# HumanCompatibleAI/overcooked_ai

Hardware: NVIDIA H100
Metric: env-steps/sec (joint transitions) (higher is better)
Workload: dtype int32

## Files before the change

### overcooked_ai_b200/csrc/ovc_b200.cu

```cuda
#include <cuda.h>
#include <cuda_runtime.h>
#include <stdint.h>
#include <stdio.h>
#include <stdlib.h>
#include <string.h>

#include "../../include/ovc_b200.h"
#include "ovc_step.cuh"

namespace ovc {

static thread_local char g_err[512] = "";

static int fail(int code, const char *msg) {
    snprintf(g_err, sizeof g_err, "%s", msg);
    return code;
}
static int fail(int code, const char *msg, long long value) {
    snprintf(g_err, sizeof g_err, "%s (got %lld)", msg, value);
    return code;
}
static int cuda_fail(cudaError_t e, const char *what) {
    snprintf(g_err, sizeof g_err, "%s: %s", what, cudaGetErrorString(e));
    return OVC_E_CUDA;
}

__device__ __forceinline__ uint32_t smem_u32(const void *p) { return (uint32_t)__cvta_generic_to_shared(p); }

__device__ __forceinline__ void mbar_init(uint64_t *bar, int count) {
    asm volatile("mbarrier.init.shared::cta.b64 [%0], %1;" ::"r"(smem_u32(bar)), "r"(count) : "memory");
    asm volatile("fence.mbarrier_init.release.cluster;" ::: "memory");
    asm volatile("fence.proxy.async.shared::cta;" ::: "memory");
}
__device__ __forceinline__ void mbar_expect_tx(uint64_t *bar, uint32_t bytes) {
    asm volatile("mbarrier.arrive.expect_tx.shared::cta.b64 _, [%0], %1;" ::"r"(smem_u32(bar)), "r"(bytes) : "memory");
}
__device__ __forceinline__ void mbar_wait(uint64_t *bar, uint32_t parity) {
    uint32_t ok;
    do {
// ... 988 lines not shown
```

### overcooked_ai_b200/csrc/ovc_encfc.cuh

```cuda
#pragma once
#include <cuda_bf16.h>
#include <type_traits>

namespace ovc {

constexpr int EL_DYN = 19;
constexpr int EL_THREADS = 1024;
constexpr int EL_MAX_LAYOUTS = 8;
constexpr int EL_MAX_MEMBERS = 64;

struct EncLinArgs {
    const ovc_layout_t *layouts;
    const int32_t *state;
    const int32_t *view_swap;
    const __nv_bfloat16 *wt;
    const float *bias;
    __nv_bfloat16 *out;
    long long n_envs;
    int n_layouts, S, W, H, horizon, n_out, n_workers;
    float neg_slope;
    int seat;
    const int32_t *rows;
    const int32_t *range;
};
// ... 65 lines not shown
    constexpr int CS = 32 * CPL;
    extern __shared__ __align__(16) char el_smem[];
    const int WH = a.W * a.H;
    const int n_rows = WH * EL_DYN;
    __nv_bfloat16 *tab = reinterpret_cast<__nv_bfloat16 *>(el_smem);
    float *bias_eff = reinterpret_cast<float *>(el_smem + (size_t)n_rows * CS * 2);
    float *urg = bias_eff + a.n_layouts * CS;
    int *cook = reinterpret_cast<int *>(urg + CS);
    int *nslots = cook + a.n_layouts * 16;
    unsigned short *srow = reinterpret_cast<unsigned short *>(nslots + a.n_layouts * 2);

    const int n_slices = a.n_out / CS;
    const __nv_bfloat16 *wt = a.wt;
    const float *bias = a.bias;
    long long r_beg = 0, r_end = a.n_envs;
    int slice = blockIdx.x % n_slices, worker = blockIdx.x / n_slices;
    if constexpr (GROUPED) {
        int bx = blockIdx.x;
        const int per = n_slices * a.n_workers, k = bx / per;
        bx -= k * per;
        wt += (size_t)k * a.W * a.H * N_PLANES * a.n_out, bias += (size_t)k * a.n_out;
        r_beg = min(max((long long)__ldg(offsets + k), 0ll), a.n_envs);
        r_end = max(min((long long)__ldg(offsets + k + 1), a.n_envs), r_beg);
        slice = bx % n_slices, worker = bx / n_slices;
    }
    const int col0 = slice * CS;
    if constexpr (ROWS) {
        r_beg = max(__ldg(a.range), 0);
        r_end = min((long long)__ldg(a.range + 1), a.n_envs);
        if (r_beg + (long long)worker * (EL_THREADS / 32) >= r_end) return;
    }
    if constexpr (MASKED) {
        if ((long long)worker * (EL_THREADS / 32) >= r_end) return;
    }
    if constexpr (GROUPED) {
        if (r_beg + (long long)worker * (EL_THREADS / 32) >= r_end) return;
    }

    unsigned char *tplane = reinterpret_cast<unsigned char *>(srow + a.n_layouts * 128);
    for (int i = threadIdx.x; i < a.n_layouts * WH; i += EL_THREADS) {
        const int l = i / WH, cell = i - l * WH, x = cell / a.H, y = cell - x * a.H;
        tplane[l * 256 + cell] = (unsigned char)((0x000F0A0E0D0C0B00ull >> ((a.layouts[l].cell[(y << 4) | x] & 7) * 8)) & 0xFF);
    }
    __syncthreads();
    {
        constexpr int CH = CS * 2 / 16;
        for (int i = threadIdx.x; i < n_rows * CH; i += EL_THREADS) {
            const int r = i / CH, c = i - r * CH;
            const int cell = r / EL_DYN, d = r - cell * EL_DYN;
            const int plane = d < 10 ? d : d + 6;
            const uint4 *src = reinterpret_cast<const uint4 *>(wt + (size_t)(cell * N_PLANES + plane) * a.n_out + col0) + c;
            reinterpret_cast<uint4 *>(tab)[i] = __ldg(src);
// ... 15 lines not shown
            if (l == a.n_layouts) urg[c] = s;
            else bias_eff[i] = s;
        }
        for (int i = threadIdx.x; i < a.n_layouts * 128; i += EL_THREADS) {
            const ovc_layout_t *L = a.layouts + (i >> 7);
            const int pb = L->slot_pos[i & 127];
            srow[i] = (unsigned short)((((pb & 15) * a.H + (pb >> 4)) * EL_DYN) & 0xFFFF);
        }
        for (int i = threadIdx.x; i < a.n_layouts * 16; i += EL_THREADS) cook[i] = a.layouts[i >> 4].cook_time[i & 15];
        for (int i = threadIdx.x; i < a.n_layouts; i += EL_THREADS) {
            nslots[2 * i] = a.layouts[i].n_slots;
            nslots[2 * i + 1] = a.layouts[i].n_pots;
        }
    }
    __syncthreads();

    const int lane = threadIdx.x & 31, warp = threadIdx.x >> 5;
    constexpr int NW = EL_THREADS / 32;
    const __nv_bfloat16 *tab_lane = tab + lane * CPL;
    const long long stride = (long long)a.n_workers * NW;
    const int max_slot_chunks = (a.S - 4 + 31) / 32;

    for (long long r = r_beg + (long long)worker * NW + warp; r < r_end; r += stride) {
        long long env, row0 = 0;
        int vmask = 3;
        if constexpr (MASKED) {
            const int entry = __ldg(list + r);
            env = entry >> 2, vmask = entry & 3;
            if (!vmask) continue;
            row0 = __ldg(first + r);
// ... 151 lines not shown
    a.out = (__nv_bfloat16 *)out, a.n_envs = n_envs, a.n_layouts = n_layouts, a.S = S, a.W = W, a.H = H, a.horizon = horizon;
    a.n_out = n_out, a.neg_slope = neg_slope, a.seat = seat, a.rows = rows, a.range = range;
    const int n_slices = n_out / (32 * cpl);
    const long long want = (n_envs + EL_THREADS / 32 - 1) / (EL_THREADS / 32);
    int workers = n_sm / n_slices;
    if (grouped) workers /= n_members;
    if (workers < 1) workers = 1;
    if (workers > want) workers = (int)want;
    a.n_workers = workers;
    const size_t smem = encode_linear_smem(cpl, n_rows, n_layouts);
    cudaError_t e;
#define OVC_LAUNCH_EL(C, ...)                                                                                                 \
    do {                                                                                                                      \
        e = cudaFuncSetAttribute(encode_linear_kernel<C, __VA_ARGS__>, cudaFuncAttributeMaxDynamicSharedMemorySize, (int)smem); \
        if (e != cudaSuccess) return cuda_fail(e, "encode_linear kernel attribute");                                          \
        encode_linear_kernel<C, __VA_ARGS__><<<(unsigned)(workers * n_slices), EL_THREADS, smem, st>>>(a);                    \
    } while (0)
#define OVC_LAUNCH_ELM(C)                                                                                                     \
    do {                                                                                                                      \
        e = cudaFuncSetAttribute(encode_linear_masked_kernel<C>, cudaFuncAttributeMaxDynamicSharedMemorySize, (int)smem);     \
        if (e != cudaSuccess) return cuda_fail(e, "encode_linear kernel attribute");                                          \
        encode_linear_masked_kernel<C><<<(unsigned)(workers * n_slices), EL_THREADS, smem, st>>>(a, list, first);             \
    } while (0)
#define OVC_LAUNCH_ELG(C)                                                                                                     \
    do {                                                                                                                      \
        e = cudaFuncSetAttribute(encode_linear_grouped_kernel<C>, cudaFuncAttributeMaxDynamicSharedMemorySize, (int)smem);    \
        if (e != cudaSuccess) return cuda_fail(e, "encode_linear kernel attribute");                                          \
        encode_linear_grouped_kernel<C><<<grid, EL_THREADS, smem, st>>>(a, offsets);                                          \
    } while (0)
#define OVC_LAUNCH_ELGM(C)                                                                                                    \
    do {                                                                                                                      \
        e = cudaFuncSetAttribute(encode_linear_grouped_masked_kernel<C>, cudaFuncAttributeMaxDynamicSharedMemorySize, (int)smem); \
        if (e != cudaSuccess) return cuda_fail(e, "encode_linear kernel attribute");                                          \
        encode_linear_grouped_masked_kernel<C><<<grid, EL_THREADS, smem, st>>>(a, list, first, offsets);                      \
    } while (0)
    if (grouped && masked) {
        const unsigned grid = (unsigned)(workers * n_slices * n_members);
        if (cpl == 8) OVC_LAUNCH_ELGM(8);
        else if (cpl == 4) OVC_LAUNCH_ELGM(4);
        else OVC_LAUNCH_ELGM(2);
    } else if (grouped) {
        const unsigned grid = (unsigned)(workers * n_slices * n_members);
        if (cpl == 8) OVC_LAUNCH_ELG(8);
        else if (cpl == 4) OVC_LAUNCH_ELG(4);
        else OVC_LAUNCH_ELG(2);
    } else if (masked) {
        if (cpl == 8) OVC_LAUNCH_ELM(8);
        else if (cpl == 4) OVC_LAUNCH_ELM(4);
        else OVC_LAUNCH_ELM(2);
// ... 2 lines not shown
        else if (cpl == 4) OVC_LAUNCH_EL(4, true, true);
        else OVC_LAUNCH_EL(2, true, true);
    } else if (seat >= 0) {
        if (cpl == 8) OVC_LAUNCH_EL(8, true);
        else if (cpl == 4) OVC_LAUNCH_EL(4, true);
        else OVC_LAUNCH_EL(2, true);
    } else {
        if (cpl == 8) OVC_LAUNCH_EL(8, false);
        else if (cpl == 4) OVC_LAUNCH_EL(4, false);
        else OVC_LAUNCH_EL(2, false);
    }
#undef OVC_LAUNCH_EL
#undef OVC_LAUNCH_ELM
#undef OVC_LAUNCH_ELG
#undef OVC_LAUNCH_ELGM
    e = cudaGetLastError();
    if (e != cudaSuccess) return cuda_fail(e, "encode_linear kernel launch");
    return OVC_OK;
}

constexpr int WG_SMEM_LIMIT = 227 * 1024;

struct EncWgradArgs {
    const ovc_layout_t *layouts;
    const int32_t *state;
    const int32_t *swap;
    const float *dz;
    float *dwt;
    long long n_rec;
    int n_layouts, S, W, H, horizon, n_out, n_workers;
    int seat;
// ... 226 lines not shown
            counter[0] = step + 1;
            __threadfence();
        }
    }
}

enum class RowMap { Identity, View, Rows, Joint };

template <bool LOGP, RowMap MAP>
__global__ void __launch_bounds__(256) sample_actions_kernel(const float *__restrict__ scores, int ld, int n_actions, long long n_rows,
                                                             unsigned long long seed, unsigned long long *counter,
                                                             int32_t *__restrict__ actions, float *__restrict__ logp,
                                                             const int32_t *__restrict__ swap, int seat, const int32_t *__restrict__ rows,
                                                             const int32_t *__restrict__ range) {
    static_assert(MAP != RowMap::Joint, "the draw has no joint-rows form");
    const unsigned long long step = *reinterpret_cast<volatile unsigned long long *>(counter);
    const long long row = (long long)blockIdx.x * blockDim.x + threadIdx.x;
    const bool in = MAP == RowMap::Rows ? row >= max(__ldg(range), 0) && row < min((long long)__ldg(range + 1), n_rows) : row < n_rows;
    if (in) {
        const float *s = scores + row * ld;
        long long g = row;
        if constexpr (MAP != RowMap::Identity) {
            const long long e = MAP == RowMap::Rows ? (long long)__ldg(rows + row) : row;
            g = 2 * e + (seat ^ (swap && swap[e] != 0));
        }
        const uint32_t c3 = (uint32_t)(step >> 32) << 1;
        const Philox4 A = philox4x32_10(seed, (uint32_t)g, (uint32_t)((unsigned long long)g >> 32), (uint32_t)step, c3);
        Philox4 B = A;
        if (n_actions > 4) B = philox4x32_10(seed, (uint32_t)g, (uint32_t)((unsigned long long)g >> 32), (uint32_t)step, c3 | 1u);
        int best = 0;
// ... 88 lines not shown
    } else if (rewards) {
        reinterpret_cast<float2 *>(rewards)[e] = make_float2(__fadd_rn((float)sp, __fmul_rn(f, (float)sh.x)), __fadd_rn((float)sp, __fmul_rn(f, (float)sh.y)));
    }
    if (dones) dones[e] = done[e] != 0;
    if constexpr (STATS)
        episode_stats_update(stats, e, n_envs, sh, __fadd_rn((float)sp, __fmul_rn(f, (float)sh.x)), __fadd_rn((float)sp, __fmul_rn(f, (float)sh.y)),
                             done[e] != 0);
}

template <bool STATS>
__global__ void __launch_bounds__(256) accumulate_returns_kernel(const int32_t *__restrict__ sparse, const int32_t *__restrict__ shaped,
                                                                 float factor, long long n_envs, long long *__restrict__ ret_sparse,
                                                                 float *__restrict__ ret_mixed, const float *__restrict__ factor_dev,
                                                                 const int32_t *__restrict__ done, float *__restrict__ rewards,
                                                                 uint8_t *__restrict__ dones, const ovc_episode_stats_t stats) {
    const long long e = (long long)blockIdx.x * blockDim.x + threadIdx.x;
    if (e >= n_envs) return;
    record_body<STATS, false>(e, sparse, shaped, factor_dev ? *factor_dev : factor, n_envs, ret_sparse, ret_mixed, done, nullptr, 0, rewards,
                              dones, stats);
}

static int sample_actions_impl(const float *scores, int ld, int n_actions, long long n_rows, unsigned long long seed,
                               unsigned long long *counter, int32_t *actions, float *logp, cudaStream_t st, RowMap map = RowMap::Identity,
                               const int32_t *swap = nullptr, int seat = 0, const int32_t *rows = nullptr, const int32_t *range = nullptr) {
    const bool listed = map == RowMap::Rows;
    if (!scores || !counter || !actions || (listed && (!rows || !range))) return fail(OVC_E_BADARG, "null pointer argument");
    if (listed && seat != 0 && seat != 1) return fail(OVC_E_BADARG, "seat must be 0 or 1", seat);
    if (n_actions < 1 || n_actions > 8 || ld < n_actions) return fail(OVC_E_BADARG, "n_actions must be 1..8 and <= ld", n_actions);
    if (n_rows < 0) return fail(OVC_E_BADARG, "negative row count");
    if (listed) {
        if ((((uintptr_t)scores | (uintptr_t)actions | (uintptr_t)logp | (uintptr_t)swap | (uintptr_t)rows | (uintptr_t)range) & 3) != 0)
            return fail(OVC_E_BADARG, "scores, actions, logp, swap, rows and range must be 4-byte aligned");
        if (((uintptr_t)counter & 7) != 0) return fail(OVC_E_BADARG, "counter must be 8-byte aligned");
    } else if (map == RowMap::View && (((uintptr_t)scores | (uintptr_t)actions | (uintptr_t)logp | (uintptr_t)swap) & 3) != 0) {
        return fail(OVC_E_BADARG, "scores, actions, logp and swap must be 4-byte aligned");
    }
    if (n_rows == 0) return OVC_OK;
    const unsigned grid = (unsigned)((n_rows + 255) / 256);
    auto kern = listed                ? (logp ? sample_actions_kernel<true, RowMap::Rows> : sample_actions_kernel<false, RowMap::Rows>)
                : map == RowMap::View ? (logp ? sample_actions_kernel<true, RowMap::View> : sample_actions_kernel<false, RowMap::View>)
                : logp                ? sample_actions_kernel<true, RowMap::Identity>
                                      : sample_actions_kernel<false, RowMap::Identity>;
    kern<<<grid, 256, 0, st>>>(scores, ld, n_actions, n_rows, seed, counter, actions, logp, swap, seat, rows, range);
    cudaError_t e = cudaGetLastError();
    if (e != cudaSuccess) return cuda_fail(e, listed ? "sample_actions_rows kernel launch" : "sample_actions kernel launch");
    return OVC_OK;
}

static int check_record_args(const int32_t *sparse, const int32_t *shaped, long long n_envs, const int32_t *done, const uint8_t *dones,
                             const ovc_episode_stats_t *stats) {
    if (!sparse || !shaped || (dones && !done)) return fail(OVC_E_BADARG, "null pointer argument");
    if (n_envs < 0) return fail(OVC_E_BADARG, "negative env count");
    if (stats) {
        const ovc_episode_stats_t &s = *stats;
        if (!done || !s.layouts || !s.state || !s.events || !s.event_counts || !s.sparse_by_agent || !s.shaped_by_agent || !s.ep_length ||
            !s.layout_id || !s.count || !s.dropped)
            return fail(OVC_E_BADARG, "null pointer argument (episode statistics)");
        if (s.capacity < 0) return fail(OVC_E_BADARG, "negative record capacity", s.capacity);
        if (s.capacity > 0 && (!s.rec_length || !s.rec_layout || !s.rec_partner_seat || !s.rec_sparse_by_agent || !s.rec_shaped_by_agent ||
// ... 3 lines not shown
        if (((uintptr_t)s.event_counts | (uintptr_t)s.rec_event_counts | (uintptr_t)s.events | (uintptr_t)s.reward_by_agent |
             (uintptr_t)s.rec_reward_by_agent) & 7)
            return fail(OVC_E_BADARG, "event and reward buffers must be 8-byte aligned");
        if (((uintptr_t)s.sparse_by_agent | (uintptr_t)s.shaped_by_agent | (uintptr_t)s.rec_sparse_by_agent | (uintptr_t)s.rec_shaped_by_agent) & 15)
            return fail(OVC_E_BADARG, "int64 sums must be 16-byte aligned");
    }
    return OVC_OK;
}

static int accumulate_returns_impl(const int32_t *sparse, const int32_t *shaped, float factor, long long n_envs, long long *ret_sparse,
                                   float *ret_mixed, const float *factor_dev, const int32_t *done, float *rewards, uint8_t *dones,
                                   const ovc_episode_stats_t *stats, cudaStream_t st) {
    if (int rc = check_record_args(sparse, shaped, n_envs, done, dones, stats)) return rc;
    if (n_envs == 0) return OVC_OK;
    const unsigned grid = (unsigned)((n_envs + 255) / 256);
    if (stats)
        accumulate_returns_kernel<true><<<grid, 256, 0, st>>>(sparse, shaped, factor, n_envs, ret_sparse, ret_mixed, factor_dev, done,
                                                              rewards, dones, *stats);
    else
        accumulate_returns_kernel<false><<<grid, 256, 0, st>>>(sparse, shaped, factor, n_envs, ret_sparse, ret_mixed, factor_dev, done,
                                                               rewards, dones, ovc_episode_stats_t{});
    cudaError_t e = cudaGetLastError();
    if (e != cudaSuccess) return cuda_fail(e, "accumulate_returns kernel launch");
    return OVC_OK;
}

template <bool STATS>
__global__ void __launch_bounds__(256) record_transition_view_kernel(const int32_t *__restrict__ sparse, const int32_t *__restrict__ shaped,
                                                                     long long n_envs, long long *__restrict__ ret_sparse,
                                                                     float *__restrict__ ret_mixed, const float *__restrict__ factor_dev,
                                                                     const int32_t *__restrict__ done, const int32_t *__restrict__ swap,
                                                                     int seat, float *__restrict__ rewards, uint8_t *__restrict__ dones,
                                                                     const ovc_episode_stats_t stats) {
    const long long e = (long long)blockIdx.x * blockDim.x + threadIdx.x;
    if (e >= n_envs) return;
    record_body<STATS, true>(e, sparse, shaped, *factor_dev, n_envs, ret_sparse, ret_mixed, done, swap, seat, rewards, dones, stats);
}

static int record_transition_view_impl(const int32_t *sparse, const int32_t *shaped, const int32_t *done, const float *factor_dev,
                                       long long n_envs, const int32_t *swap, int seat, float *rewards, uint8_t *dones,
                                       long long *ret_sparse, float *ret_mixed, const ovc_episode_stats_t *stats, cudaStream_t st) {
    if (!factor_dev || !rewards) return fail(OVC_E_BADARG, "null pointer argument");
    if (int rc = check_record_args(sparse, shaped, n_envs, done, dones, stats)) return rc;
    if (seat != 0 && seat != 1) return fail(OVC_E_BADARG, "seat must be 0 or 1", seat);
    if (((uintptr_t)rewards | (uintptr_t)swap) & 3) return fail(OVC_E_BADARG, "rewards and swap must be 4-byte aligned");
    if (n_envs == 0) return OVC_OK;
    const unsigned grid = (unsigned)((n_envs + 255) / 256);
    if (stats)
        record_transition_view_kernel<true><<<grid, 256, 0, st>>>(sparse, shaped, n_envs, ret_sparse, ret_mixed, factor_dev, done, swap,
                                                                  seat, rewards, dones, *stats);
    else
        record_transition_view_kernel<false><<<grid, 256, 0, st>>>(sparse, shaped, n_envs, ret_sparse, ret_mixed, factor_dev, done, swap,
                                                                   seat, rewards, dones, ovc_episode_stats_t{});
    cudaError_t e = cudaGetLastError();
    if (e != cudaSuccess) return cuda_fail(e, "record_transition_view kernel launch");
    return OVC_OK;
}

template <bool STATS, bool ONE_VIEW>
__global__ void __launch_bounds__(256) record_transition_dense_kernel(const int32_t *__restrict__ sparse, const int32_t *__restrict__ shaped,
                                                                      const float *__restrict__ dense, long long n_envs,
                                                                      long long *__restrict__ ret_sparse, float *__restrict__ ret_mixed,
                                                                      const float *__restrict__ factor_dev, const int32_t *__restrict__ done,
                                                                      float *__restrict__ rewards, uint8_t *__restrict__ dones,
                                                                      const ovc_episode_stats_t stats) {
    const long long e = (long long)blockIdx.x * blockDim.x + threadIdx.x;
    if (e >= n_envs) return;
    const float f = *factor_dev;
    const int sp = sparse[e];
    const float fd = __fmul_rn(f, dense[e]);
    const float r = __fadd_rn((float)sp, fd);
    if (ret_sparse) ret_sparse[e] += sp;
    if (ret_mixed) ret_mixed[e] = __fadd_rn(__fadd_rn(__fadd_rn(ret_mixed[e], (float)sp), fd), fd);
    if (rewards) {
        if (ONE_VIEW) rewards[e] = r;
        else reinterpret_cast<float2 *>(rewards)[e] = make_float2(r, r);
    }
    if (dones) dones[e] = done[e] != 0;
    if constexpr (STATS) episode_stats_update(stats, e, n_envs, reinterpret_cast<const int2 *>(shaped)[e], r, r, done[e] != 0);
}

static int record_transition_dense_impl(const int32_t *sparse, const int32_t *shaped, const float *dense, const int32_t *done,
                                        const float *factor_dev, long long n_envs, int one_view, float *rewards, uint8_t *dones,
                                        long long *ret_sparse, float *ret_mixed, const ovc_episode_stats_t *stats, cudaStream_t st) {
    if (!factor_dev || !dense) return fail(OVC_E_BADARG, "null pointer argument");
    if (int rc = check_record_args(sparse, shaped, n_envs, done, dones, stats)) return rc;
    if (one_view != 0 && one_view != 1) return fail(OVC_E_BADARG, "one_view must be 0 or 1", one_view);
    if (((uintptr_t)dense & 3) || ((uintptr_t)rewards & (one_view ? 3 : 7)))
        return fail(OVC_E_BADARG, "dense must be 4-byte aligned, rewards 4-byte (one view) or 8-byte (two rows)");
    if (n_envs == 0) return OVC_OK;
    const unsigned grid = (unsigned)((n_envs + 255) / 256);
    const ovc_episode_stats_t s = stats ? *stats : ovc_episode_stats_t{};
    auto kern = stats ? (one_view ? record_transition_dense_kernel<true, true> : record_transition_dense_kernel<true, false>)
                      : (one_view ? record_transition_dense_kernel<false, true> : record_transition_dense_kernel<false, false>);
    kern<<<grid, 256, 0, st>>>(sparse, shaped, dense, n_envs, ret_sparse, ret_mixed, factor_dev, done, rewards, dones, s);
    cudaError_t e = cudaGetLastError();
    if (e != cudaSuccess) return cuda_fail(e, "record_transition_dense kernel launch");
    return OVC_OK;
}

constexpr int GAE_THREADS = 128;
constexpr int GAE_UNROLL = 16;

__device__ __forceinline__ float gae_step(float a, float r, float v, float nv, float nt, float gamma, float gl) {
    const float d = __fsub_rn(__fadd_rn(r, __fmul_rn(__fmul_rn(gamma, nv), nt)), v);
    return __fadd_rn(d, __fmul_rn(__fmul_rn(gl, nt), a));
}
__device__ __forceinline__ float2 gae_step(float2 a, float2 r, float2 v, float2 nv, float nt, float gamma, float gl) {
    return make_float2(gae_step(a.x, r.x, v.x, nv.x, nt, gamma, gl), gae_step(a.y, r.y, v.y, nv.y, nt, gamma, gl));
}
__device__ __forceinline__ float gae_target(float a, float v) { return __fadd_rn(a, v); }
// ... 53 lines not shown
```

### overcooked_ai_b200/csrc/ovc_tail.cuh

```cuda
#pragma once
#include <cuda_bf16.h>

namespace ovc {

constexpr int PT_THREADS = 512;
constexpr int PT_H = 64;
constexpr int PT_HS = 80;
constexpr int PT_NOUT = 8;

struct PolicyTailArgs {
    const __nv_bfloat16 *x;
    const __nv_bfloat16 *w_first;
    const float *b_first;
    const __nv_bfloat16 *w_hidden;
    const float *b_hidden;
    const __nv_bfloat16 *w_heads;
    const float *b_heads;
    long long n_rows;
    int n_hidden, n_actions;
    float in_slope, slope;
    unsigned long long seed;
    unsigned long long *counter;
    int32_t *actions;
    float *values;
// ... 206 lines not shown
        const int best = draw_row<LOGP>(s0, s1, p.seed, step, d, p.n_actions, lane, t, lp);
        if (in) {
            if (t == 0) p.actions[d] = best;
            if constexpr (LOGP) if (t == 0) p.logp[o] = lp;
            if (p.values && t == (p.n_actions >> 1)) p.values[o] = (p.n_actions & 1) ? s1 : s0;
        }
    }
}

template <int KS2, RowMap MAP, bool LOGP, bool HIDDEN = false>
__global__ void __launch_bounds__(PT_THREADS, 1) policy_tail_kernel(const PolicyTailArgs p) {
    static_assert(!HIDDEN || (MAP == RowMap::Identity && !LOGP), "the hidden form has no draw");
    constexpr int K0 = 32 * KS2;
    extern __shared__ __align__(16) char pt_smem[];

    const unsigned long long step = HIDDEN ? 0ull : *reinterpret_cast<volatile unsigned long long *>(p.counter);
    const TailSmem w = tail_weights_to_smem<K0, PT_THREADS>(pt_smem, p);
    __syncthreads();

    const int lane = threadIdx.x & 31, warp = threadIdx.x >> 5, g = lane >> 2, t = lane & 3;
    constexpr bool RANGED = MAP == RowMap::Rows || MAP == RowMap::Joint;
    using Row = typename std::conditional<RANGED, int, long long>::type;
    Row r_beg = 0, r_end = p.n_rows;
    if constexpr (RANGED) {
        r_beg = max(__ldg(p.range), 0);
        r_end = max((int)min((long long)__ldg(p.range + 1), p.n_rows), r_beg);
    }
    const Row n_tiles = (r_end - r_beg + 15) / 16;
    for (Row tile = (Row)blockIdx.x * (PT_THREADS / 32) + warp; tile < n_tiles; tile += (Row)gridDim.x * (PT_THREADS / 32)) {
        const Row r0 = r_beg + tile * 16 + g, r1 = r0 + 8;
        if constexpr (HIDDEN) {
            unsigned a[4][4];
// ... 12 lines not shown
        }
    }
    if constexpr (!HIDDEN) advance_step(p.counter, step);
}

constexpr int PT_MAX_MEMBERS = 64;
constexpr int PTG_THREADS = 384;

template <int KS2, bool LOGP, RowMap MAP = RowMap::Identity>
__global__ void __launch_bounds__(PTG_THREADS, 1) policy_tail_grouped_kernel(const PolicyTailArgs p) {
    static_assert(MAP == RowMap::Identity || (MAP == RowMap::Joint && LOGP), "the grouped forms: Identity, or Joint with logp");
    constexpr int K0 = 32 * KS2;
    extern __shared__ __align__(16) char pt_smem[];
    __shared__ int tile0[PT_MAX_MEMBERS + 1], rbeg[PT_MAX_MEMBERS], rend[PT_MAX_MEMBERS];

    const unsigned long long step = *reinterpret_cast<volatile unsigned long long *>(p.counter);
    if (threadIdx.x == 0) {
        int n = 0;
        for (int k = 0; k < p.n_members; k++) {
            const int lo = max(__ldg(p.offsets + k), 0), hi = max((int)min((long long)__ldg(p.offsets + k + 1), p.n_rows), lo);
            tile0[k] = n, rbeg[k] = lo, rend[k] = hi;
            n += (hi - lo + 15) / 16;
        }
        tile0[p.n_members] = n;
    }
    __syncthreads();
    const int total = tile0[p.n_members];
    const int t_lo = (int)((long long)blockIdx.x * total / gridDim.x), t_hi = (int)((long long)(blockIdx.x + 1) * total / gridDim.x);
    const int lane = threadIdx.x & 31, warp = threadIdx.x >> 5, g = lane >> 2, t = lane & 3;
    int tb = t_lo;
// ... 39 lines not shown
    cudaGetDevice(&dev);
    cudaDeviceGetAttribute(&n_sm, cudaDevAttrMultiProcessorCount, dev);
    const int threads = grouped ? PTG_THREADS : PT_THREADS;
    const size_t smem = tail_smem_bytes(k0, a.n_hidden) + 16;
    const long long n_tiles = (a.n_rows + 15) / 16 + (grouped ? a.n_members : 0), want = (n_tiles + threads / 32 - 1) / (threads / 32);
    const unsigned grid = (unsigned)(want < n_sm ? want : n_sm);
    PolicyTailKernel kern = nullptr;
#define OVC_PT_CASE(KS2) \
    case KS2: kern = policy_tail_pick<KS2>(map, a.logp, hid, grouped); break;
    switch (k0 / 32) {
        OVC_PT_CASE(1) OVC_PT_CASE(2) OVC_PT_CASE(3) OVC_PT_CASE(4) OVC_PT_CASE(5) OVC_PT_CASE(6) OVC_PT_CASE(7) OVC_PT_CASE(8)
    }
#undef OVC_PT_CASE
    cudaError_t e = cudaFuncSetAttribute(kern, cudaFuncAttributeMaxDynamicSharedMemorySize, (int)smem);
    if (e != cudaSuccess) return cuda_fail(e, grouped ? "policy_tail_grouped kernel attribute" : "policy_tail kernel attribute");
    kern<<<grid, threads, smem, st>>>(a);
    e = cudaGetLastError();
    if (e != cudaSuccess) return cuda_fail(e, grouped ? "policy_tail_grouped kernel launch" : "policy_tail kernel launch");
    return OVC_OK;
}

static int policy_tail_grouped_impl(const PolicyTailArgs &a, int k0, cudaStream_t st, RowMap map = RowMap::Identity) {
    if (!a.x || !a.w_first || !a.b_first || !a.w_heads || !a.b_heads || !a.counter || !a.actions || !a.offsets ||
        (a.n_hidden > 0 && (!a.w_hidden || !a.b_hidden)) || (map == RowMap::Joint && (!a.rows || !a.logp)))
        return fail(OVC_E_BADARG, "null pointer argument");
    if ((((uintptr_t)a.x | (uintptr_t)a.w_first | (uintptr_t)a.w_hidden | (uintptr_t)a.w_heads) & 15) != 0)
        return fail(OVC_E_BADARG, "x and the weight tables must be 16-byte aligned");
    if ((((uintptr_t)a.b_first | (uintptr_t)a.b_hidden | (uintptr_t)a.b_heads | (uintptr_t)a.scores | (uintptr_t)a.counter) & 7) != 0)
        return fail(OVC_E_BADARG, "biases, scores and counter must be 8-byte aligned");
    if ((((uintptr_t)a.actions | (uintptr_t)a.values | (uintptr_t)a.logp | (uintptr_t)a.offsets) & 3) != 0)
        return fail(OVC_E_BADARG, "actions, values, logp and offsets must be 4-byte aligned");
    if (((uintptr_t)a.rows & 3) != 0) return fail(OVC_E_BADARG, "jrow must be 4-byte aligned");
// ... 32 lines not shown
```

### overcooked_ai_b200/csrc/ovc_wide.cuh

```cuda
#pragma once
#include <cuda_bf16.h>

namespace ovc {

constexpr int WL_BM = 128, WL_BK = 64, WL_K0 = 512, WL_N1 = 512, WL_N2 = 160;
constexpr int WL_NC = 128;
constexpr int WL_KC = WL_K0 / WL_BK;
constexpr int WL_CHUNKS = WL_N1 / WL_NC;
constexpr int WL_THREADS = 384;
constexpr int WL_STAGES = 4;
constexpr uint32_t WL_A_BYTES = WL_BM * WL_BK * 2;
constexpr uint32_t WL_B1_BYTES = WL_NC * WL_BK * 2;
constexpr uint32_t WL_STAGE = WL_A_BYTES + WL_B1_BYTES;
constexpr uint32_t WL_B2_BOX = WL_N2 * WL_BK * 2;
constexpr uint32_t WL_B2_STAGE = (WL_NC / WL_BK) * WL_B2_BOX;
constexpr uint32_t WL_TILE_BYTES = WL_STAGES * WL_STAGE + 2 * WL_B2_STAGE;
constexpr uint32_t WL_SMEM = 1024 + WL_TILE_BYTES + (WL_N1 + WL_N2) * 4 + 128;
static_assert(WL_SMEM <= 227 * 1024, "one CTA per SM within the opt-in shared memory of sm_90");

struct WideArgs {
    const float *b1, *b2;
    __nv_bfloat16 *z2;
    long long m;
    float slope;
// ... 85 lines not shown
        : "memory");
}

__device__ __forceinline__ uint32_t leaky_bf16x2(float x0, float x1, float slope) {
    const __nv_bfloat162 h = __floats2bfloat162_rn(fmaxf(x0, x0 * slope), fmaxf(x1, x1 * slope));
    return *reinterpret_cast<const uint32_t *>(&h);
}

template <bool RANGE = false, bool GROUPED = false>
__global__ void __launch_bounds__(WL_THREADS, 1)
wide_layers_kernel(const __grid_constant__ CUtensorMap map_a0, const __grid_constant__ CUtensorMap map_w1,
                   const __grid_constant__ CUtensorMap map_w2, const WideArgs p) {
    static_assert(!(RANGE && GROUPED), "a grouped launch reads its members' offsets, not a range");
    long long r_beg = 0, r_end = p.m;
    int n_tiles = p.n_tiles;
    if constexpr (RANGE) {
        r_beg = max(__ldg(p.range), 0);
        r_end = max(min((long long)__ldg(p.range + 1), p.m), r_beg);
        n_tiles = (int)((r_end - r_beg + WL_BM - 1) / WL_BM);
    }
    __shared__ int g_tile0[GROUPED ? WL_MAX_MEMBERS + 1 : 1], g_rbeg[GROUPED ? WL_MAX_MEMBERS : 1], g_rend[GROUPED ? WL_MAX_MEMBERS : 1];
    if constexpr (GROUPED) {
        if (threadIdx.x == 0) {
            int t = 0;
            for (int k = 0; k < p.n_tiles; k++) {
                const int lo = (int)min(max((long long)__ldg(p.range + k), 0ll), p.m);
                const int hi = (int)max(min((long long)__ldg(p.range + k + 1), p.m), (long long)lo);
                g_tile0[k] = t, g_rbeg[k] = lo, g_rend[k] = hi;
                t += (hi - lo + WL_BM - 1) / WL_BM;
            }
            g_tile0[p.n_tiles] = t;
        }
        __syncthreads();
        n_tiles = g_tile0[p.n_tiles];
    }
    auto tile_member = [&](int i, int &k, long long &m0, long long &end) {
        k = 0;
        while (g_tile0[k + 1] <= i) k++;
        m0 = g_rbeg[k] + (long long)(i - g_tile0[k]) * WL_BM, end = g_rend[k];
    };
    extern __shared__ char wl_raw[];
    char *tile = reinterpret_cast<char *>((reinterpret_cast<uintptr_t>(wl_raw) + 1023) & ~(uintptr_t)1023);
    char *w2_tile = tile + WL_STAGES * WL_STAGE;
    float *bias1 = reinterpret_cast<float *>(tile + WL_TILE_BYTES);
    float *bias2 = bias1 + WL_N1;
    uint64_t *bars = reinterpret_cast<uint64_t *>(bias2 + WL_N2);
    uint64_t *full = bars, *empty = bars + WL_STAGES, *w2_full = bars + 2 * WL_STAGES, *w2_empty = w2_full + 2;

    const int warp = threadIdx.x >> 5, lane = threadIdx.x & 31;

    if (threadIdx.x == 0) {
        for (int i = 0; i < WL_STAGES; i++) mbar_init(full + i, 1), mbar_init(empty + i, 8);
        for (int i = 0; i < 2; i++) mbar_init(w2_full + i, 1), mbar_init(w2_empty + i, 8);
        prefetch_tmap(&map_a0), prefetch_tmap(&map_w1), prefetch_tmap(&map_w2);
    }
    if constexpr (!GROUPED) {
        for (int i = threadIdx.x; i < WL_N1; i += WL_THREADS) bias1[i] = p.b1[i];
        for (int i = threadIdx.x; i < WL_N2; i += WL_THREADS) bias2[i] = p.b2[i];
    }
    __syncthreads();

    if (warp >= 8) {
        regs_dealloc<40>();
        if (warp == 8 && lane == 0) {
            int it1 = 0, it2 = 0;
            for (int tile_i = blockIdx.x; tile_i < n_tiles; tile_i += gridDim.x) {
                int m0 = (int)(r_beg + tile_i * WL_BM), wk = 0;
                if constexpr (GROUPED) {
                    long long gm0, gend;
                    tile_member(tile_i, wk, gm0, gend);
                    m0 = (int)gm0;
                }
                for (int n = 0; n < WL_CHUNKS; n++) {
                    for (int c = 0; c < WL_KC; c++, it1++) {
                        const int s = it1 % WL_STAGES, u = it1 / WL_STAGES;
// ... 117 lines not shown
    if (!rc) rc = make_tmap_bf16(&mw1, w1, (long long)n_members * WL_N1, WL_K0, WL_NC);
    if (!rc) rc = make_tmap_bf16(&mw2, w2, (long long)n_members * WL_N2, WL_N1, WL_N2);
    if (rc) return rc;
    void (*kern)(const CUtensorMap, const CUtensorMap, const CUtensorMap, const WideArgs) =
        grouped ? wide_layers_kernel<false, true> : range ? wide_layers_kernel<true> : wide_layers_kernel<false>;
    cudaError_t e = cudaFuncSetAttribute(kern, cudaFuncAttributeMaxDynamicSharedMemorySize, (int)WL_SMEM);
    if (e != cudaSuccess) return cuda_fail(e, "wide_layers kernel attribute");
    WideArgs p;
    int dev = 0, n_sm = 0;
    cudaGetDevice(&dev);
    cudaDeviceGetAttribute(&n_sm, cudaDevAttrMultiProcessorCount, dev);
    p.b1 = b1, p.b2 = b2, p.z2 = (__nv_bfloat16 *)z2, p.m = m, p.slope = slope, p.range = range;
    p.n_tiles = grouped ? n_members : (int)((m + WL_BM - 1) / WL_BM);
    const long long most = (m + WL_BM - 1) / WL_BM + (grouped ? n_members : 0);
    const unsigned grid = (unsigned)(most < n_sm ? most : n_sm);
    kern<<<grid, WL_THREADS, WL_SMEM, st>>>(ma, mw1, mw2, p);
    e = cudaGetLastError();
    if (e != cudaSuccess) return cuda_fail(e, "wide_layers kernel launch");
    return OVC_OK;
}

}
```

### overcooked_ai_b200/selfplay.py

```python
import copy
import functools
from types import SimpleNamespace

import numpy as np
import torch
import torch.nn as nn
import torch.nn.functional as F

from . import _native
from .batched import EpisodeRecords, EpisodeStats


class RllibShapedCNN(nn.Module):
    def __init__(self, width, height, in_planes=26, num_filters=25, hidden=64, num_hidden_layers=3, num_actions=6):
        super().__init__()
        self.conv_initial = nn.Conv2d(in_planes, num_filters, 5, padding=2)
        self.conv_0 = nn.Conv2d(num_filters, num_filters, 3, padding=1)
        self.conv_1 = nn.Conv2d(num_filters, num_filters, 3, padding=0)
        flat = num_filters * (width - 2) * (height - 2)
        dims = [flat] + [hidden] * num_hidden_layers
        self.dense = nn.ModuleList([nn.Linear(dims[i], dims[i + 1]) for i in range(num_hidden_layers)])
        self.logits = nn.Linear(hidden, num_actions)
        self.value = nn.Linear(hidden, 1)

# ... 531 lines not shown
    s = torch.cuda.Stream(dev)
    s.wait_stream(torch.cuda.current_stream(dev))
    with torch.cuda.stream(s):
        warm_up()
    torch.cuda.current_stream(dev).wait_stream(s)
    graph = torch.cuda.CUDAGraph()
    with torch.cuda.graph(graph):
        body()
    for t, v in zip(live, saved):
        t.copy_(v)
    return graph


GROUPED_K9_MIN_MEMBERS = 4


def _check_members(members, most, kinds, count_msg, kind_msg):
    assert 1 <= len(members) <= most, count_msg
    for m in members:
        assert isinstance(m, kinds) and not isinstance(m, RllibLSTMShapedCNN), kind_msg


class _Rollout(object):

    _pair_play = False

    def _init_rollout(self, env, learner, use_graph, reward_shaping_factor, episode_capacity, max_seq_len):
        N, dev = env.n_envs, env.device
        self.use_graph = use_graph
        self.actions = torch.zeros((N, 2), dtype=torch.int32, device=dev)
        self.ret_sparse = torch.zeros(N, dtype=torch.int64, device=dev)
        self.factor = float(reward_shaping_factor)
        self._factor = torch.full((1,), self.factor, dtype=torch.float32, device=dev)
        self.stats = EpisodeStats(env)
        self.episodes = EpisodeRecords(env, episode_capacity, members=self.population, pairs=self._pair_play)
        self.max_seq_len = int(max_seq_len)
        assert self.max_seq_len >= 1
        self.graph = None
        self._collect_graphs = {}
        self._batches = {}
        self._boot_counter = torch.zeros(2, dtype=torch.int64, device=dev)
        self._boot_actions = torch.zeros((N, 2), dtype=torch.int32, device=dev)
        if learner.lstm:
            self._h_boot, self._c_boot = torch.empty_like(learner.h), torch.empty_like(learner.c)

    @property
    def reward_shaping_factor(self):
        return self.factor

    @reward_shaping_factor.setter
    def reward_shaping_factor(self, value):
        self.factor = float(value)
        self._factor.fill_(self.factor)
# ... 8 lines not shown
        assert self._pop is not None and self._pop._thresholds is not None, "member_weights: a population drawn per episode"
        self._pop.weights = value

    @property
    def member(self):
        return self._member if self._pop is None else self._pop.member

    def _assign_seats(self, done):
        self.env.assign_partners(self.partner_seat, self._bc_factor, self._seat_counter, seed=self.seed ^ PARTNER_SEAT_SALT, done=done)

    def _capture(self, warm_up, body):
        live = [self.env.state, self.ret_sparse] + self.stats.state_tensors() + self.episodes.tensors() + self._live()
        return _capture_graph(self.env, live, warm_up, body)

    def run(self, n_steps):
        if self.use_graph and self.graph is None:
            def warm_up():
                for _ in range(3):
                    self._transition()
            self.graph = self._capture(warm_up, self._transition)
        step = self._transition if self.graph is None else self.graph.replay
        for _ in range(n_steps):
            step()
        return n_steps * self.env.n_envs

    def _collect_window(self, b, n_steps, gamma, lam):
        b.episodes.clear()
        for t in range(n_steps):
            self._transition(b, t)
        self._bootstrap(b)
        gae = self.env.gae_view if b.one_view else self.env.gae
        gae(b.rewards, b.values, b.dones, b.last_values, gamma, lam, b.advantages, b.value_targets)

    def collect(self, n_steps, gamma, lam, keep_logits=False):
        assert self.env.auto_reset, "collect() needs an auto_reset environment: a window runs across episode ends"
        key = (int(n_steps), bool(keep_logits))
        b = self._batches.get(key)
        if b is None:
# ... 710 lines not shown
```

Baseline: 77.18 billion.

## Chain policy kernels with programmatic dependent launch and batch graph replays

Launches the encoder, wide-layer, policy-tail, sampling and record kernels with programmatic stream serialization. Each kernel now loads its weights into shared memory, then waits on the predecessor through griddepcontrol before reading dependent data, so prologues overlap the previous kernel's tail. The run loop also captures a graph of sixteen transitions and replays it, cutting per-replay launch overhead. Row-range reads and early exits move after the wait, which adds a risk of ordering bugs if any dependent read happens before the wait.

```diff
diff --git a/overcooked_ai_b200/csrc/ovc_b200.cu b/overcooked_ai_b200/csrc/ovc_b200.cu
--- a/overcooked_ai_b200/csrc/ovc_b200.cu
+++ b/overcooked_ai_b200/csrc/ovc_b200.cu
@@ -5,6 +5,8 @@
 #include <stdlib.h>
 #include <string.h>
 
+#include <utility>
+
 #include "../../include/ovc_b200.h"
 #include "ovc_step.cuh"
 
@@ -23,6 +25,30 @@
 static int cuda_fail(cudaError_t e, const char *what) {
     snprintf(g_err, sizeof g_err, "%s: %s", what, cudaGetErrorString(e));
     return OVC_E_CUDA;
+}
+
+#define OVC_PDL_K7 1
+#define OVC_PDL_K9 2
+#define OVC_PDL_K8 4
+#define OVC_PDL_RECORD 8
+#ifndef OVC_POLICY_PDL
+#define OVC_POLICY_PDL (OVC_PDL_K7 | OVC_PDL_K9 | OVC_PDL_K8 | OVC_PDL_RECORD)
+#endif
+
+__device__ __forceinline__ void chain_wait() { asm volatile("griddepcontrol.wait;" ::: "memory"); }
+__device__ __forceinline__ void chain_release() { asm volatile("griddepcontrol.launch_dependents;" ::: "memory"); }
+
+template <int KERNEL, class... P, class... A>
+static cudaError_t chain_launch(void (*kern)(P...), dim3 grid, dim3 block, size_t smem, cudaStream_t st, A &&...args) {
+    cudaLaunchConfig_t cfg;
+    memset(&cfg, 0, sizeof cfg);
+    cfg.gridDim = grid, cfg.blockDim = block, cfg.dynamicSmemBytes = smem, cfg.stream = st;
+    cudaLaunchAttribute attr[1];
+    attr[0].id = cudaLaunchAttributeProgrammaticStreamSerialization;
+    attr[0].val.programmaticStreamSerializationAllowed = 1;
+    cfg.attrs = attr;
+    cfg.numAttrs = (OVC_POLICY_PDL & KERNEL) ? 1 : 0;
+    return cudaLaunchKernelEx(&cfg, kern, std::forward<A>(args)...);
 }
 
 __device__ __forceinline__ uint32_t smem_u32(const void *p) { return (uint32_t)__cvta_generic_to_shared(p); }
diff --git a/overcooked_ai_b200/csrc/ovc_encfc.cuh b/overcooked_ai_b200/csrc/ovc_encfc.cuh
--- a/overcooked_ai_b200/csrc/ovc_encfc.cuh
+++ b/overcooked_ai_b200/csrc/ovc_encfc.cuh
@@ -103,28 +103,16 @@
     const __nv_bfloat16 *wt = a.wt;
     const float *bias = a.bias;
     long long r_beg = 0, r_end = a.n_envs;
-    int slice = blockIdx.x % n_slices, worker = blockIdx.x / n_slices;
+    int slice = blockIdx.x % n_slices, worker = blockIdx.x / n_slices, member = 0;
     if constexpr (GROUPED) {
         int bx = blockIdx.x;
-        const int per = n_slices * a.n_workers, k = bx / per;
-        bx -= k * per;
-        wt += (size_t)k * a.W * a.H * N_PLANES * a.n_out, bias += (size_t)k * a.n_out;
-        r_beg = min(max((long long)__ldg(offsets + k), 0ll), a.n_envs);
-        r_end = max(min((long long)__ldg(offsets + k + 1), a.n_envs), r_beg);
+        const int per = n_slices * a.n_workers;
+        member = bx / per;
+        bx -= member * per;
+        wt += (size_t)member * a.W * a.H * N_PLANES * a.n_out, bias += (size_t)member * a.n_out;
         slice = bx % n_slices, worker = bx / n_slices;
     }
     const int col0 = slice * CS;
-    if constexpr (ROWS) {
-        r_beg = max(__ldg(a.range), 0);
-        r_end = min((long long)__ldg(a.range + 1), a.n_envs);
-        if (r_beg + (long long)worker * (EL_THREADS / 32) >= r_end) return;
-    }
-    if constexpr (MASKED) {
-        if ((long long)worker * (EL_THREADS / 32) >= r_end) return;
-    }
-    if constexpr (GROUPED) {
-        if (r_beg + (long long)worker * (EL_THREADS / 32) >= r_end) return;
-    }
 
     unsigned char *tplane = reinterpret_cast<unsigned char *>(srow + a.n_layouts * 128);
     for (int i = threadIdx.x; i < a.n_layouts * WH; i += EL_THREADS) {
@@ -170,6 +158,17 @@
         }
     }
     __syncthreads();
+    chain_wait();
+    chain_release();
+    if constexpr (GROUPED) {
+        r_beg = min(max((long long)__ldg(offsets + member), 0ll), a.n_envs);
+        r_end = max(min((long long)__ldg(offsets + member + 1), a.n_envs), r_beg);
+    }
+    if constexpr (ROWS) {
+        r_beg = max(__ldg(a.range), 0);
+        r_end = min((long long)__ldg(a.range + 1), a.n_envs);
+    }
+    if (r_beg + (long long)worker * (EL_THREADS / 32) >= r_end) return;
 
     const int lane = threadIdx.x & 31, warp = threadIdx.x >> 5;
     constexpr int NW = EL_THREADS / 32;
@@ -351,25 +350,25 @@
     do {                                                                                                                      \
         e = cudaFuncSetAttribute(encode_linear_kernel<C, __VA_ARGS__>, cudaFuncAttributeMaxDynamicSharedMemorySize, (int)smem); \
         if (e != cudaSuccess) return cuda_fail(e, "encode_linear kernel attribute");                                          \
-        encode_linear_kernel<C, __VA_ARGS__><<<(unsigned)(workers * n_slices), EL_THREADS, smem, st>>>(a);                    \
+        e = chain_launch<OVC_PDL_K7>(encode_linear_kernel<C, __VA_ARGS__>, (unsigned)(workers * n_slices), EL_THREADS, smem, st, a); \
     } while (0)
 #define OVC_LAUNCH_ELM(C)                                                                                                     \
     do {                                                                                                                      \
         e = cudaFuncSetAttribute(encode_linear_masked_kernel<C>, cudaFuncAttributeMaxDynamicSharedMemorySize, (int)smem);     \
         if (e != cudaSuccess) return cuda_fail(e, "encode_linear kernel attribute");                                          \
-        encode_linear_masked_kernel<C><<<(unsigned)(workers * n_slices), EL_THREADS, smem, st>>>(a, list, first);             \
+        e = chain_launch<OVC_PDL_K7>(encode_linear_masked_kernel<C>, (unsigned)(workers * n_slices), EL_THREADS, smem, st, a, list, first); \
     } while (0)
 #define OVC_LAUNCH_ELG(C)                                                                                                     \
     do {                                                                                                                      \
         e = cudaFuncSetAttribute(encode_linear_grouped_kernel<C>, cudaFuncAttributeMaxDynamicSharedMemorySize, (int)smem);    \
         if (e != cudaSuccess) return cuda_fail(e, "encode_linear kernel attribute");                                          \
-        encode_linear_grouped_kernel<C><<<grid, EL_THREADS, smem, st>>>(a, offsets);                                          \
+        e = chain_launch<OVC_PDL_K7>(encode_linear_grouped_kernel<C>, grid, EL_THREADS, smem, st, a, offsets);               \
     } while (0)
 #define OVC_LAUNCH_ELGM(C)                                                                                                    \
     do {                                                                                                                      \
         e = cudaFuncSetAttribute(encode_linear_grouped_masked_kernel<C>, cudaFuncAttributeMaxDynamicSharedMemorySize, (int)smem); \
         if (e != cudaSuccess) return cuda_fail(e, "encode_linear kernel attribute");                                          \
-        encode_linear_grouped_masked_kernel<C><<<grid, EL_THREADS, smem, st>>>(a, list, first, offsets);                      \
+        e = chain_launch<OVC_PDL_K7>(encode_linear_grouped_masked_kernel<C>, grid, EL_THREADS, smem, st, a, list, first, offsets); \
     } while (0)
     if (grouped && masked) {
         const unsigned grid = (unsigned)(workers * n_slices * n_members);
@@ -402,7 +401,6 @@
 #undef OVC_LAUNCH_ELM
 #undef OVC_LAUNCH_ELG
 #undef OVC_LAUNCH_ELGM
-    e = cudaGetLastError();
     if (e != cudaSuccess) return cuda_fail(e, "encode_linear kernel launch");
     return OVC_OK;
 }
@@ -659,6 +657,8 @@
                                                              const int32_t *__restrict__ swap, int seat, const int32_t *__restrict__ rows,
                                                              const int32_t *__restrict__ range) {
     static_assert(MAP != RowMap::Joint, "the draw has no joint-rows form");
+    chain_wait();
+    chain_release();
     const unsigned long long step = *reinterpret_cast<volatile unsigned long long *>(counter);
     const long long row = (long long)blockIdx.x * blockDim.x + threadIdx.x;
     const bool in = MAP == RowMap::Rows ? row >= max(__ldg(range), 0) && row < min((long long)__ldg(range + 1), n_rows) : row < n_rows;
@@ -777,6 +777,8 @@
                                                                  float *__restrict__ ret_mixed, const float *__restrict__ factor_dev,
                                                                  const int32_t *__restrict__ done, float *__restrict__ rewards,
                                                                  uint8_t *__restrict__ dones, const ovc_episode_stats_t stats) {
+    chain_release();
+    chain_wait();
     const long long e = (long long)blockIdx.x * blockDim.x + threadIdx.x;
     if (e >= n_envs) return;
     record_body<STATS, false>(e, sparse, shaped, factor_dev ? *factor_dev : factor, n_envs, ret_sparse, ret_mixed, done, nullptr, 0, rewards,
@@ -804,8 +806,8 @@
                 : map == RowMap::View ? (logp ? sample_actions_kernel<true, RowMap::View> : sample_actions_kernel<false, RowMap::View>)
                 : logp                ? sample_actions_kernel<true, RowMap::Identity>
                                       : sample_actions_kernel<false, RowMap::Identity>;
-    kern<<<grid, 256, 0, st>>>(scores, ld, n_actions, n_rows, seed, counter, actions, logp, swap, seat, rows, range);
-    cudaError_t e = cudaGetLastError();
+    const cudaError_t e = chain_launch<OVC_PDL_K8>(kern, grid, 256, 0, st, scores, ld, n_actions, n_rows, seed, counter, actions, logp,
+                                                   swap, seat, rows, range);
     if (e != cudaSuccess) return cuda_fail(e, listed ? "sample_actions_rows kernel launch" : "sample_actions kernel launch");
     return OVC_OK;
 }
@@ -839,13 +841,9 @@
     if (int rc = check_record_args(sparse, shaped, n_envs, done, dones, stats)) return rc;
     if (n_envs == 0) return OVC_OK;
     const unsigned grid = (unsigned)((n_envs + 255) / 256);
-    if (stats)
-        accumulate_returns_kernel<true><<<grid, 256, 0, st>>>(sparse, shaped, factor, n_envs, ret_sparse, ret_mixed, factor_dev, done,
-                                                              rewards, dones, *stats);
-    else
-        accumulate_returns_kernel<false><<<grid, 256, 0, st>>>(sparse, shaped, factor, n_envs, ret_sparse, ret_mixed, factor_dev, done,
-                                                               rewards, dones, ovc_episode_stats_t{});
-    cudaError_t e = cudaGetLastError();
+    const cudaError_t e = chain_launch<OVC_PDL_RECORD>(stats ? accumulate_returns_kernel<true> : accumulate_returns_kernel<false>, grid, 256, 0,
+                                                       st, sparse, shaped, factor, n_envs, ret_sparse, ret_mixed, factor_dev, done, rewards,
+                                                       dones, stats ? *stats : ovc_episode_stats_t{});
     if (e != cudaSuccess) return cuda_fail(e, "accumulate_returns kernel launch");
     return OVC_OK;
 }
@@ -857,6 +855,8 @@
                                                                      const int32_t *__restrict__ done, const int32_t *__restrict__ swap,
                                                                      int seat, float *__restrict__ rewards, uint8_t *__restrict__ dones,
                                                                      const ovc_episode_stats_t stats) {
+    chain_release();
+    chain_wait();
     const long long e = (long long)blockIdx.x * blockDim.x + threadIdx.x;
     if (e >= n_envs) return;
     record_body<STATS, true>(e, sparse, shaped, *factor_dev, n_envs, ret_sparse, ret_mixed, done, swap, seat, rewards, dones, stats);
@@ -871,13 +871,9 @@
     if (((uintptr_t)rewards | (uintptr_t)swap) & 3) return fail(OVC_E_BADARG, "rewards and swap must be 4-byte aligned");
     if (n_envs == 0) return OVC_OK;
     const unsigned grid = (unsigned)((n_envs + 255) / 256);
-    if (stats)
-        record_transition_view_kernel<true><<<grid, 256, 0, st>>>(sparse, shaped, n_envs, ret_sparse, ret_mixed, factor_dev, done, swap,
-                                                                  seat, rewards, dones, *stats);
-    else
-        record_transition_view_kernel<false><<<grid, 256, 0, st>>>(sparse, shaped, n_envs, ret_sparse, ret_mixed, factor_dev, done, swap,
-                                                                   seat, rewards, dones, ovc_episode_stats_t{});
-    cudaError_t e = cudaGetLastError();
+    const cudaError_t e = chain_launch<OVC_PDL_RECORD>(stats ? record_transition_view_kernel<true> : record_transition_view_kernel<false>,
+                                                       grid, 256, 0, st, sparse, shaped, n_envs, ret_sparse, ret_mixed, factor_dev, done,
+                                                       swap, seat, rewards, dones, stats ? *stats : ovc_episode_stats_t{});
     if (e != cudaSuccess) return cuda_fail(e, "record_transition_view kernel launch");
     return OVC_OK;
 }
@@ -889,6 +885,8 @@
                                                                       const float *__restrict__ factor_dev, const int32_t *__restrict__ done,
                                                                       float *__restrict__ rewards, uint8_t *__restrict__ dones,
                                                                       const ovc_episode_stats_t stats) {
+    chain_release();
+    chain_wait();
     const long long e = (long long)blockIdx.x * blockDim.x + threadIdx.x;
     if (e >= n_envs) return;
     const float f = *factor_dev;
@@ -918,8 +916,8 @@
     const ovc_episode_stats_t s = stats ? *stats : ovc_episode_stats_t{};
     auto kern = stats ? (one_view ? record_transition_dense_kernel<true, true> : record_transition_dense_kernel<true, false>)
                       : (one_view ? record_transition_dense_kernel<false, true> : record_transition_dense_kernel<false, false>);
-    kern<<<grid, 256, 0, st>>>(sparse, shaped, dense, n_envs, ret_sparse, ret_mixed, factor_dev, done, rewards, dones, s);
-    cudaError_t e = cudaGetLastError();
+    const cudaError_t e = chain_launch<OVC_PDL_RECORD>(kern, grid, 256, 0, st, sparse, shaped, dense, n_envs, ret_sparse, ret_mixed,
+                                                       factor_dev, done, rewards, dones, s);
     if (e != cudaSuccess) return cuda_fail(e, "record_transition_dense kernel launch");
     return OVC_OK;
 }
diff --git a/overcooked_ai_b200/csrc/ovc_tail.cuh b/overcooked_ai_b200/csrc/ovc_tail.cuh
--- a/overcooked_ai_b200/csrc/ovc_tail.cuh
+++ b/overcooked_ai_b200/csrc/ovc_tail.cuh
@@ -244,8 +244,10 @@
     constexpr int K0 = 32 * KS2;
     extern __shared__ __align__(16) char pt_smem[];
 
+    const TailSmem w = tail_weights_to_smem<K0, PT_THREADS>(pt_smem, p);
+    chain_wait();
+    chain_release();
     const unsigned long long step = HIDDEN ? 0ull : *reinterpret_cast<volatile unsigned long long *>(p.counter);
-    const TailSmem w = tail_weights_to_smem<K0, PT_THREADS>(pt_smem, p);
     __syncthreads();
 
     const int lane = threadIdx.x & 31, warp = threadIdx.x >> 5, g = lane >> 2, t = lane & 3;
@@ -288,6 +290,8 @@
     extern __shared__ __align__(16) char pt_smem[];
     __shared__ int tile0[PT_MAX_MEMBERS + 1], rbeg[PT_MAX_MEMBERS], rend[PT_MAX_MEMBERS];
 
+    chain_wait();
+    chain_release();
     const unsigned long long step = *reinterpret_cast<volatile unsigned long long *>(p.counter);
     if (threadIdx.x == 0) {
         int n = 0;
@@ -357,8 +361,7 @@
 #undef OVC_PT_CASE
     cudaError_t e = cudaFuncSetAttribute(kern, cudaFuncAttributeMaxDynamicSharedMemorySize, (int)smem);
     if (e != cudaSuccess) return cuda_fail(e, grouped ? "policy_tail_grouped kernel attribute" : "policy_tail kernel attribute");
-    kern<<<grid, threads, smem, st>>>(a);
-    e = cudaGetLastError();
+    e = chain_launch<OVC_PDL_K8>(kern, grid, threads, smem, st, a);
     if (e != cudaSuccess) return cuda_fail(e, grouped ? "policy_tail_grouped kernel launch" : "policy_tail kernel launch");
     return OVC_OK;
 }
diff --git a/overcooked_ai_b200/csrc/ovc_wide.cuh b/overcooked_ai_b200/csrc/ovc_wide.cuh
--- a/overcooked_ai_b200/csrc/ovc_wide.cuh
+++ b/overcooked_ai_b200/csrc/ovc_wide.cuh
@@ -123,26 +123,7 @@
     static_assert(!(RANGE && GROUPED), "a grouped launch reads its members' offsets, not a range");
     long long r_beg = 0, r_end = p.m;
     int n_tiles = p.n_tiles;
-    if constexpr (RANGE) {
-        r_beg = max(__ldg(p.range), 0);
-        r_end = max(min((long long)__ldg(p.range + 1), p.m), r_beg);
-        n_tiles = (int)((r_end - r_beg + WL_BM - 1) / WL_BM);
-    }
     __shared__ int g_tile0[GROUPED ? WL_MAX_MEMBERS + 1 : 1], g_rbeg[GROUPED ? WL_MAX_MEMBERS : 1], g_rend[GROUPED ? WL_MAX_MEMBERS : 1];
-    if constexpr (GROUPED) {
-        if (threadIdx.x == 0) {
-            int t = 0;
-            for (int k = 0; k < p.n_tiles; k++) {
-                const int lo = (int)min(max((long long)__ldg(p.range + k), 0ll), p.m);
-                const int hi = (int)max(min((long long)__ldg(p.range + k + 1), p.m), (long long)lo);
-                g_tile0[k] = t, g_rbeg[k] = lo, g_rend[k] = hi;
-                t += (hi - lo + WL_BM - 1) / WL_BM;
-            }
-            g_tile0[p.n_tiles] = t;
-        }
-        __syncthreads();
-        n_tiles = g_tile0[p.n_tiles];
-    }
     auto tile_member = [&](int i, int &k, long long &m0, long long &end) {
         k = 0;
         while (g_tile0[k + 1] <= i) k++;
@@ -167,7 +148,27 @@
         for (int i = threadIdx.x; i < WL_N1; i += WL_THREADS) bias1[i] = p.b1[i];
         for (int i = threadIdx.x; i < WL_N2; i += WL_THREADS) bias2[i] = p.b2[i];
     }
+    chain_wait();
+    chain_release();
+    if constexpr (RANGE) {
+        r_beg = max(__ldg(p.range), 0);
+        r_end = max(min((long long)__ldg(p.range + 1), p.m), r_beg);
+        n_tiles = (int)((r_end - r_beg + WL_BM - 1) / WL_BM);
+    }
+    if constexpr (GROUPED) {
+        if (threadIdx.x == 0) {
+            int t = 0;
+            for (int k = 0; k < p.n_tiles; k++) {
+                const int lo = (int)min(max((long long)__ldg(p.range + k), 0ll), p.m);
+                const int hi = (int)max(min((long long)__ldg(p.range + k + 1), p.m), (long long)lo);
+                g_tile0[k] = t, g_rbeg[k] = lo, g_rend[k] = hi;
+                t += (hi - lo + WL_BM - 1) / WL_BM;
+            }
+            g_tile0[p.n_tiles] = t;
+        }
+    }
     __syncthreads();
+    if constexpr (GROUPED) n_tiles = g_tile0[p.n_tiles];
 
     if (warp >= 8) {
         regs_dealloc<40>();
@@ -315,8 +316,7 @@
     p.n_tiles = grouped ? n_members : (int)((m + WL_BM - 1) / WL_BM);
     const long long most = (m + WL_BM - 1) / WL_BM + (grouped ? n_members : 0);
     const unsigned grid = (unsigned)(most < n_sm ? most : n_sm);
-    kern<<<grid, WL_THREADS, WL_SMEM, st>>>(ma, mw1, mw2, p);
-    e = cudaGetLastError();
+    e = chain_launch<OVC_PDL_K9>(kern, grid, WL_THREADS, WL_SMEM, st, ma, mw1, mw2, p);
     if (e != cudaSuccess) return cuda_fail(e, "wide_layers kernel launch");
     return OVC_OK;
 }
diff --git a/overcooked_ai_b200/selfplay.py b/overcooked_ai_b200/selfplay.py
--- a/overcooked_ai_b200/selfplay.py
+++ b/overcooked_ai_b200/selfplay.py
@@ -569,6 +569,8 @@
 
 GROUPED_K9_MIN_MEMBERS = 4
 
+RUN_GRAPH_TRANSITIONS = 16
+
 
 def _check_members(members, most, kinds, count_msg, kind_msg):
     assert 1 <= len(members) <= most, count_msg
@@ -592,6 +594,7 @@
         self.max_seq_len = int(max_seq_len)
         assert self.max_seq_len >= 1
         self.graph = None
+        self._run_graph = None
         self._collect_graphs = {}
         self._batches = {}
         self._boot_counter = torch.zeros(2, dtype=torch.int64, device=dev)
@@ -630,14 +633,25 @@
         return _capture_graph(self.env, live, warm_up, body)
 
     def run(self, n_steps):
+        def warm_up():
+            for _ in range(3):
+                self._transition()
         if self.use_graph and self.graph is None:
-            def warm_up():
-                for _ in range(3):
+            self.graph = self._capture(warm_up, self._transition)
+        if self.graph is None:
+            for _ in range(n_steps):
+                self._transition()
+            return n_steps * self.env.n_envs
+        k = RUN_GRAPH_TRANSITIONS
+        if n_steps >= k and self._run_graph is None:
+            def body():
+                for _ in range(k):
                     self._transition()
-            self.graph = self._capture(warm_up, self._transition)
-        step = self._transition if self.graph is None else self.graph.replay
-        for _ in range(n_steps):
-            step()
+            self._run_graph = self._capture(warm_up, body)
+        for _ in range(n_steps // k):
+            self._run_graph.replay()
+        for _ in range(n_steps % k):
+            self.graph.replay()
         return n_steps * self.env.n_envs
 
     def _collect_window(self, b, n_steps, gamma, lam):
```

Result: no change. 77.20 billion (median of 6 runs) (+0.0%).
